# OSU-Bee-Lab/buzzdetect

Hardware: AMD Instinct MI355X
Metric: yamnet_windows_per_s (higher is better)
Workload: dtype f32 (split-f16x3 MFMA products, f32 accumulate)

## Files before the change

### buzzdetect_amd/csrc/bd_device.h

```cpp
#pragma once

#include "bd_internal.h"

#include <mutex>
#include <type_traits>
#ifdef BD_KERNEL_TRACE
#include <cstdio>
#include <cstdlib>
#endif

namespace bd {

namespace {

typedef float f32x16 __attribute__((ext_vector_type(16)));
typedef float v2f __attribute__((ext_vector_type(2)));
typedef float v4f __attribute__((ext_vector_type(4)));
typedef unsigned v4u __attribute__((ext_vector_type(4)));
typedef unsigned u32x2 __attribute__((ext_vector_type(2)));
typedef _Float16 f16x2 __attribute__((ext_vector_type(2)));
typedef _Float16 f16x4 __attribute__((ext_vector_type(4)));
typedef _Float16 f16x8 __attribute__((ext_vector_type(8)));

constexpr float kF16Max = 65504.0f;
__device__ __forceinline__ float range_of(float m, float4 v) {
    return fmaxf(fmaxf(m, fabsf(v.x)), fmaxf(fmaxf(fabsf(v.y), fabsf(v.z)), fabsf(v.w)));
}
__device__ __forceinline__ float range_of(float m, v4f v) {
    return fmaxf(fmaxf(m, fabsf(v.x)), fmaxf(fmaxf(fabsf(v.y), fabsf(v.z)), fabsf(v.w)));
}
__device__ __forceinline__ void range_report(float m, unsigned* __restrict__ flag) {
    if (flag && !(m <= kF16Max)) *flag = 1u;
}

__device__ __forceinline__ int swz64(int row, int slot) { return row * 64 + ((slot ^ ((row >> 2) & 3)) << 4); }

__device__ __forceinline__ void split_f16(float x, float y, float z, float w, f16x4& hi, f16x4& lo) {
    const f16x2 h0 = {(_Float16)x, (_Float16)y}, h1 = {(_Float16)z, (_Float16)w};
    f16x2 l0, l1;
    asm("v_fma_mixlo_f16 %0, %1, -1.0, %2 op_sel:[0,0,0] op_sel_hi:[1,0,0]" : "=v"(l0) : "v"(h0), "v"(x));
    asm("v_fma_mixhi_f16 %0, %1, -1.0, %2 op_sel:[1,0,0] op_sel_hi:[1,0,0]" : "+v"(l0) : "v"(h0), "v"(y));
    asm("v_fma_mixlo_f16 %0, %1, -1.0, %2 op_sel:[0,0,0] op_sel_hi:[1,0,0]" : "=v"(l1) : "v"(h1), "v"(z));
    asm("v_fma_mixhi_f16 %0, %1, -1.0, %2 op_sel:[1,0,0] op_sel_hi:[1,0,0]" : "+v"(l1) : "v"(h1), "v"(w));
    hi[0] = h0[0]; hi[1] = h0[1]; hi[2] = h1[0]; hi[3] = h1[1];
    lo[0] = l0[0]; lo[1] = l0[1]; lo[2] = l1[0]; lo[3] = l1[1];
}
__device__ __forceinline__ void split_f16(v4f a, f16x4& hi, f16x4& lo) { split_f16(a.x, a.y, a.z, a.w, hi, lo); }

constexpr int kTrRowBytes = 192, kTrHalfBytes = 32 * kTrRowBytes, kTrSlotBytes = 2 * kTrHalfBytes;
__host__ __device__ constexpr int tr_image_off(int half, int k, int chunk) {
    return half * kTrHalfBytes + k * kTrRowBytes + ((chunk ^ ((k >> 1) & 7)) << 3);
}
__host__ __device__ constexpr int tr_read_k(int s, int h, int r, int q) { return 16 * s + 8 * h + 4 * r + q; }
__host__ __device__ constexpr int tr_read_chunk(int i, int gp, int p) { return 8 * i + 4 * gp + p; }
constexpr bool tr_image_is_bijection() {
    bool seen[kTrSlotBytes / 8] = {};
    for (int half = 0; half < 2; ++half)
        for (int k = 0; k < 32; ++k)
            for (int t = 0; t < 24; ++t) {
                const int o = tr_image_off(half, k, t);
                if (o < 0 || o >= kTrSlotBytes || o % 8 || seen[o / 8]) return false;
                seen[o / 8] = true;
            }
    return true;
}
constexpr bool tr_image_writes_conflict_free() {
    for (int half = 0; half < 2; ++half)
        for (int a = 0; a < 2; ++a)
            for (int t = 0; t < 24; ++t) {
                unsigned banks = 0;
                for (int l = 0; l < 16; ++l)
                    for (int d = 0; d < 2; ++d) {
                        const unsigned b = 1u << ((tr_image_off(half, 16 * a + l, t) / 4 + d) % 32);
                        if (banks & b) return false;
                        banks |= b;
                    }
            }
    return true;
}
constexpr bool tr_image_reads_conflict_free() {
    for (int half = 0; half < 2; ++half)
        for (int i = 0; i < 3; ++i)
            for (int s = 0; s < 2; ++s)
                for (int h = 0; h < 2; ++h)
                    for (int r = 0; r < 2; ++r) {
                        unsigned long long banks = 0;
                        for (int gp = 0; gp < 2; ++gp)
                            for (int q = 0; q < 4; ++q)
                                for (int p = 0; p < 4; ++p)
                                    for (int d = 0; d < 2; ++d) {
                                        const unsigned long long b =
                                            1ull << ((tr_image_off(half, tr_read_k(s, h, r, q), tr_read_chunk(i, gp, p)) / 4 + d) % 64);
                                        if (banks & b) return false;
                                        banks |= b;
                                    }
                    }
    return true;
}
static_assert(tr_image_is_bijection(), "every (half, k, chunk) has its own 8 bytes of the slot, and they fill it");
static_assert(tr_image_writes_conflict_free(), "a lane group of the publication meets no bank twice");
static_assert(tr_image_reads_conflict_free(), "a lane half of the transposed read meets no bank twice");
__device__ __forceinline__ int tr_read_lane_off(int lane) {
    const int g = lane >> 4, q = (lane >> 2) & 3, p = lane & 3;
    return tr_image_off(0, tr_read_k(0, g >> 1, 0, q), tr_read_chunk(0, g & 1, p));
}
__host__ __device__ constexpr int tr_read_next(int off) { return (off ^ 16) + 4 * kTrRowBytes; }
constexpr bool tr_read_next_holds() {
    for (int lane = 0; lane < 64; ++lane) {
        const int g = lane >> 4, q = (lane >> 2) & 3, p = lane & 3;
        if (tr_read_next(tr_image_off(0, tr_read_k(0, g >> 1, 0, q), tr_read_chunk(0, g & 1, p))) !=
            tr_image_off(0, tr_read_k(0, g >> 1, 1, q), tr_read_chunk(0, g & 1, p)))
            return false;
        for (int s = 0; s < 2; ++s)
            for (int i = 0; i < 3; ++i)
                for (int r = 0; r < 2; ++r)
                    if (tr_image_off(0, tr_read_k(s, g >> 1, r, q), tr_read_chunk(i, g & 1, p)) !=
                        tr_image_off(0, tr_read_k(0, g >> 1, r, q), tr_read_chunk(0, g & 1, p)) + 16 * s * kTrRowBytes + 64 * i)
                        return false;
    }
    return true;
}
static_assert(tr_read_next_holds(), "the reader's immediates");
__device__ __forceinline__ f16x8 tr_read_frag(const char* p0, const char* p1) {
    typedef short s16x4 __attribute__((ext_vector_type(4)));
    typedef __attribute__((address_space(3))) s16x4* lds4;
    const s16x4 a = __builtin_amdgcn_ds_read_tr16_b64_v4i16((lds4)p0), b = __builtin_amdgcn_ds_read_tr16_b64_v4i16((lds4)p1);
    return __builtin_bit_cast(f16x8, __builtin_shufflevector(a, b, 0, 1, 2, 3, 4, 5, 6, 7));
}

__device__ __forceinline__ unsigned pw_lds_addr(const void* p) {
    return (unsigned)(unsigned long long)(__attribute__((address_space(3))) const void*)p;
}
template <int OFFSET>
__device__ __forceinline__ f16x8 pw_lds_frag(unsigned addr) {
    f16x8 v;
    asm volatile("ds_read_b128 %0, %1 offset:%2" : "=v"(v) : "v"(addr), "n"(OFFSET) : "memory");
    return v;
}
__device__ __forceinline__ void pw_lds_store64(unsigned addr, f16x4 v) {
    asm volatile("ds_write_b64 %0, %1" ::"v"(addr), "v"(v) : "memory");
}
__device__ __forceinline__ f16x8 pw_landed(f16x8 v) {
    asm volatile("" : "+v"(v));
    return v;
}
template <int N>
__device__ __forceinline__ void pw_lds_wait() {
    asm volatile("s_waitcnt lgkmcnt(%0)" ::"n"(N) : "memory");
}
template <int I, int E, typename F>
__device__ __forceinline__ void static_for_pw(F&& f) {
    if constexpr (I < E) {
        f(std::integral_constant<int, I>{});
        static_for_pw<I + 1, E>(f);
    }
}
template <int K16, int V, int R>
struct PwResSchedule {
    static constexpr int split_at(int q) {
        for (int j = 0; j < V; ++j)
            if (q == j * K16 / (V > 0 ? V : 1) + 1) return j;
        return -1;
    }
    static constexpr int issued_at_step(int u) { return (u + 2 < K16 ? R : 0) + (split_at(u) >= 0 ? R : 0); }
    static constexpr int pending(int q) {
        int upto_wait = 2 * R;
        for (int u = 0; u <= q; ++u) upto_wait += issued_at_step(u);
        int through_read = q < 2 ? R * (q + 1) : 2 * R;
        if (q >= 2) {
            for (int u = 0; u < q - 2; ++u) through_read += issued_at_step(u);
            through_read += R;
        }
        return upto_wait - through_read;
    }
};

constexpr int kMaxDevices = 64;
template <auto Kernel>
void allow_dynamic_lds(int bytes) {
    static std::once_flag once[kMaxDevices];
    int dev = 0;
    (void)hipGetDevice(&dev);
    std::call_once(once[dev & (kMaxDevices - 1)], [&] {
        (void)hipFuncSetAttribute(reinterpret_cast<const void*>(Kernel), hipFuncAttributeMaxDynamicSharedMemorySize, bytes);
    });
}

#ifdef BD_KERNEL_TRACE
constexpr int kTraceStamps = 128;
template <typename Kernel, typename Launch, typename... Args>
const unsigned long long* traced_launch(char key, Kernel kernel, int lds_bytes, hipStream_t stream, int per_group, int id1,
                                        bool* printed, Launch&& launch, const char* legend, Args... args) {
    const char* tr = getenv("BD_WS_TRACE");
    if (!tr || tr[0] != key) return nullptr;
    static unsigned long long* dbg = nullptr;
    static unsigned long long h[kTraceStamps];
    static int shots = 0;
    if (!dbg) (void)hipMalloc(&dbg, sizeof(h));
    (void)hipFuncSetAttribute(reinterpret_cast<const void*>(kernel), hipFuncAttributeMaxDynamicSharedMemorySize, lds_bytes);
    (void)hipMemsetAsync(dbg, 0, sizeof(h), stream);
    launch(dbg);
    (void)hipStreamSynchronize(stream);
    (void)hipMemcpy(h, dbg, sizeof(h), hipMemcpyDeviceToHost);
    const bool print = ++shots == 8;
    if (printed) *printed = print;
    if (print)
        for (int w = 0; w < 2; ++w) {
            fprintf(stderr, "[trace] ");
            fprintf(stderr, legend, w ? id1 : 0, args...);
            for (int i = 1; i < per_group && h[w * per_group + i]; ++i) fprintf(stderr, " %llu", h[w * per_group + i] - h[w * per_group + i - 1]);
            fprintf(stderr, "\n");
        }
    return h;
}
#endif

}

}
```

### buzzdetect_amd/csrc/l4window.hip

```cpp
#include "bd_device.h"

namespace bd {

namespace {

template <bool PLAIN, bool PLANES>
__global__ __launch_bounds__(768) void l4_window_kernel(
    const float* __restrict__ X, const float* __restrict__ dw_w, const float* __restrict__ dw_b,
    const _Float16* __restrict__ Wfhi, const _Float16* __restrict__ Wflo, const float* __restrict__ pw_u,
    const float* __restrict__ pw_b,
    const float* __restrict__ ndw_w, const float* __restrict__ ndw_b, float* __restrict__ out, int windows,
    unsigned* __restrict__ range_flag, const _Float16* __restrict__ W3fhi, const _Float16* __restrict__ W3flo,
    const float* __restrict__ pw3_u, const float* __restrict__ pw3_b) {
    constexpr int H = 24, W = 16, C = 128, K16 = 8, STEPS = H / 2;
    constexpr int COL_B = C * 4;
    constexpr int ROW_B = (W + 1) * COL_B;
    constexpr int RING0 = COL_B;
    constexpr int A0 = RING0 + 8 * ROW_B;
    constexpr int A_HALF = 32 * 2 * C, A_BUF = 2 * A_HALF;
    constexpr int T5 = A0 + 2 * A_BUF;
    constexpr int O5 = T5 + C * 12 * 4;
    constexpr int O5_ROW = (W / 2) * C * 4, O5_BUF = 2 * O5_ROW;
    constexpr int PL0 = O5 + 2 * O5_BUF;
    constexpr int PL_B = 8192, PL_HALF = 4096;
    constexpr int W3L = PL0 + 2 * PL_B;
    constexpr size_t WIN_IN = (size_t)H * W * C, WIN_OUT = (size_t)STEPS * (W / 2) * C;
    static_assert(A0 % 512 == 0, "fragment addresses are formed by XOR");
    static_assert((2 * STEPS) % 8 == 0 && STEPS % 2 == 0, "ring slots and buffer parities carry over from window to window");
    extern __shared__ __attribute__((aligned(1024))) char smem_raw[];
    char* const smem = smem_raw;
    const int tid = threadIdx.x, lane = tid & 63;
    const int wave = __builtin_amdgcn_readfirstlane(tid >> 6);
    const int b = blockIdx.x, G = gridDim.x;
    if (b >= windows) return;
    const int NT = STEPS * ((windows - b + G - 1) / G);

    for (int i = tid; i < 9 * 32; i += 768) {
        const int z = i >> 5;
        *reinterpret_cast<v4f*>(smem + (z == 0 ? 0 : RING0 + (z - 1) * ROW_B + W * COL_B) + (i & 31) * 16) = v4f{0.f, 0.f, 0.f, 0.f};
    }
    for (int i = tid; i < 10 * C; i += 768) {
        const int t = i / C, c = i - t * C;
        reinterpret_cast<float*>(smem + T5)[c * 12 + t] = t < 9 ? ndw_w[t * C + c] : ndw_b[c];
    }
    float rmax = 0.0f;

    if (wave < 4) {
        const int frow = lane & 31, fh = lane >> 5;
        const int c4 = tid & 31, col_lo = tid >> 5;
        const float* const xt = X + (size_t)b * WIN_IN + (size_t)col_lo * C + c4 * 4;
        char* const ring_t = smem + RING0 + col_lo * COL_B + c4 * 16;
        v4f rs[2][4];
#define BD_L4_LOAD(DST, J)                                                                                \
    {                                                                                                     \
        const int i_ = (J) / STEPS, j_ = (J) - i_ * STEPS;                                                \
        const float* const src_ = xt + (size_t)i_ * G * WIN_IN + (size_t)j_ * (2 * W * C);                \
        _Pragma("unroll") for (int u = 0; u < 4; ++u)                                                     \
            DST[u] = *reinterpret_cast<const v4f*>(src_ + ((u >> 1) * W + 8 * (u & 1)) * C);              \
    }
#define BD_L4_STORE(SRC, J)                                                                               \
    _Pragma("unroll") for (int u = 0; u < 4; ++u)                                                         \
        *reinterpret_cast<v4f*>(ring_t + ((2 * (J) + (u >> 1)) & 7) * ROW_B + 8 * (u & 1) * COL_B) = SRC[u];
        const char* const pt = reinterpret_cast<const char*>(X) + (size_t)b * STEPS * PL_B + tid * 16;
        v4f rp[2], rq[2];
#define BD_L4_PLOAD(DST, J)                                                                               \
    {                                                                                                     \
        const int i_ = (J) / STEPS, j_ = (J) - i_ * STEPS;                                                \
        const char* const src_ = pt + ((size_t)i_ * G * STEPS + j_) * PL_B;                               \
        DST[0] = *reinterpret_cast<const v4f*>(src_);                                                     \
        if constexpr (!PLAIN) DST[1] = *reinterpret_cast<const v4f*>(src_ + PL_HALF);                     \
    }
#define BD_L4_PSTORE(SRC, J)                                                                              \
    {                                                                                                     \
        char* const st_ = smem + PL0 + ((J) & 1) * PL_B + tid * 16;                                       \
        *reinterpret_cast<v4f*>(st_) = SRC[0];                                                            \
        if constexpr (!PLAIN) *reinterpret_cast<v4f*>(st_ + PL_HALF) = SRC[1];                            \
    }
        if constexpr (PLANES) {
            BD_L4_PLOAD(rp, 0)
            BD_L4_PLOAD(rq, 1)
        } else {
            BD_L4_LOAD(rs[0], 0)
            BD_L4_LOAD(rs[1], 1)
        }
        f16x8 bh[K16], bl[K16];
#pragma unroll
        for (int q = 0; q < K16; ++q) {
            const size_t frag = ((size_t)(wave * K16 + q) * 64 + lane) * 8;
            bh[q] = *reinterpret_cast<const f16x8*>(Wfhi + frag);
            if constexpr (!PLAIN) bl[q] = *reinterpret_cast<const f16x8*>(Wflo + frag);
        }
        const int ncol = 32 * wave + frow;
        const float bcol = pw_b[ncol], ucol = pw_u[ncol];
        f16x8 w3h[PLANES ? 4 : 1];
        char* const w3l = smem + W3L + (wave * 4 * 64 + lane) * 16;
        float u3 = 0.0f, b3 = 0.0f;
        if constexpr (PLANES) {
#pragma unroll
            for (int q = 0; q < 4; ++q) {
                const size_t frag = ((size_t)(wave * 4 + q) * 64 + lane) * 8;
                w3h[q] = *reinterpret_cast<const f16x8*>(W3fhi + frag);
                if constexpr (!PLAIN) *reinterpret_cast<f16x8*>(w3l + q * 1024) = *reinterpret_cast<const f16x8*>(W3flo + frag);
            }
            u3 = pw3_u[ncol];
            b3 = pw3_b[ncol];
        }
        typedef const __attribute__((address_space(3))) f16x8* lptrh;
        unsigned pl_a[2];
        pl_a[0] = pw_lds_addr(smem) + (unsigned)(PL0 + frow * 64 + ((fh ^ ((frow >> 2) & 3)) << 4));
        pl_a[1] = pl_a[0] ^ 32u;
        asm("" : "+v"(pl_a[0]), "+v"(pl_a[1]));
        auto pw3 = [&](auto stage_c, int J) {
            constexpr int stage = decltype(stage_c)::value;
            f32x16 acc3;
#pragma unroll
            for (int r = 0; r < 16; ++r) acc3[r] = 0.0f;
#pragma unroll
            for (int q = 0; q < 4; ++q) {
                const unsigned a = pl_a[q & 1] + (unsigned)(stage * PL_B + (q >> 1) * 2048);
                const f16x8 ah = *(lptrh)(size_t)a;
                if constexpr (!PLAIN) {
                    const f16x8 al = *(lptrh)(size_t)(a + PL_HALF);
                    acc3 = __builtin_amdgcn_mfma_f32_32x32x16_f16(al, w3h[q], acc3, 0, 0, 0);
                    acc3 = __builtin_amdgcn_mfma_f32_32x32x16_f16(ah, *reinterpret_cast<const f16x8*>(w3l + q * 1024), acc3, 0, 0, 0);
                }
                acc3 = __builtin_amdgcn_mfma_f32_32x32x16_f16(ah, w3h[q], acc3, 0, 0, 0);
            }
            char* const rw = smem + RING0 + ncol * 4;
#pragma unroll
            for (int r = 0; r < 16; ++r) {
                const int m = 4 * fh + (r & 3) + 8 * (r >> 2);
                *reinterpret_cast<float*>(rw + ((2 * J + (m >> 4)) & 7) * ROW_B + (m & 15) * COL_B) = fmaxf(fmaf(acc3[r], u3, b3), 0.0f);
            }
        };
        const float* const t5 = reinterpret_cast<const float*>(smem + T5) + ncol * 12;
        float acc5[4] = {0.0f, 0.0f, 0.0f, 0.0f};
        float* const o5 = reinterpret_cast<float*>(smem + O5) + (2 * fh) * C + ncol;
        int s5 = 0;
        if constexpr (PLANES) {
            BD_L4_PSTORE(rp, 0)
            BD_L4_PSTORE(rq, 1)
            BD_L4_PLOAD(rp, 2)
            BD_L4_PLOAD(rq, 3)
        } else {
            BD_L4_STORE(rs[0], 0)
            BD_L4_STORE(rs[1], 1)
            BD_L4_LOAD(rs[0], 2)
            BD_L4_LOAD(rs[1], 3)
        }
#pragma unroll
        for (int q = 0; q < K16; ++q) {
            bh[q] = pw_landed(bh[q]);
            if constexpr (!PLAIN) bl[q] = pw_landed(bl[q]);
        }
        if constexpr (PLANES) {
            __syncthreads();
            pw3(std::integral_constant<int, 0>{}, 0);
            __syncthreads();
            BD_L4_PSTORE(rp, 2)
            rp[0] = rq[0];
            rp[1] = rq[1];
            pw3(std::integral_constant<int, 1>{}, 1);
        }
        const unsigned fr0 = pw_lds_addr(smem) + (unsigned)(A0 + frow * 2 * C + ((fh ^ (frow & 15)) << 4));
        __syncthreads();
        auto step = [&](auto pc, int k) {
            constexpr int p = decltype(pc)::value;
            f32x16 acc;
            if (k >= 1 && k <= NT) {
                const unsigned ab = fr0 + (unsigned)((p ^ 1) * A_BUF);
                using S = PwResSchedule<K16, 0, PLAIN ? 1 : 2>;
#pragma unroll
                for (int e = 0; e < 16; ++e) acc[e] = 0.0f;
                f16x8 fa[3][2];
#pragma unroll
                for (int q = 0; q < 2; ++q) {
                    fa[q][0] = pw_lds_frag<0>(ab ^ (q << 5));
                    if constexpr (!PLAIN) fa[q][1] = pw_lds_frag<A_HALF>(ab ^ (q << 5));
                }
                static_for_pw<0, K16>([&](auto qi) {
                    constexpr int q = decltype(qi)::value;
                    if constexpr (q + 2 < K16) {
                        fa[(q + 2) % 3][0] = pw_lds_frag<0>(ab ^ ((q + 2) << 5));
                        if constexpr (!PLAIN) fa[(q + 2) % 3][1] = pw_lds_frag<A_HALF>(ab ^ ((q + 2) << 5));
                    }
                    pw_lds_wait<S::pending(q)>();
                    const f16x8 ah = pw_landed(fa[q % 3][0]);
                    if constexpr (!PLAIN) {
                        const f16x8 al = pw_landed(fa[q % 3][1]);
                        acc = __builtin_amdgcn_mfma_f32_32x32x16_f16(al, bh[q], acc, 0, 0, 0);
                        acc = __builtin_amdgcn_mfma_f32_32x32x16_f16(ah, bl[q], acc, 0, 0, 0);
                    }
                    acc = __builtin_amdgcn_mfma_f32_32x32x16_f16(ah, bh[q], acc, 0, 0, 0);
                });
            }
            if constexpr (PLANES) {
                if (k + 3 < NT) BD_L4_PSTORE(rp, k + 3)
                if (k + 4 < NT) BD_L4_PLOAD(rp, k + 4)
            } else {
                if (k + 2 < NT) { BD_L4_STORE(rs[p], k + 2) }
                if (k + 4 < NT) BD_L4_LOAD(rs[p], k + 4)
            }
            if (k >= 1 && k <= NT) {
                float y[2][8], nb[2][2];
                const v4f t5a = *reinterpret_cast<const v4f*>(t5), t5b = *reinterpret_cast<const v4f*>(t5 + 4), t5c = *reinterpret_cast<const v4f*>(t5 + 8);
                const float w5[9] = {t5a.x, t5a.y, t5a.z, t5a.w, t5b.x, t5b.y, t5b.z, t5b.w, t5c.x};
                const float b5 = t5c.y;
#pragma unroll
                for (int e = 0; e < 16; ++e) y[e >> 3][e & 7] = fmaxf(fmaf(acc[e], ucol, bcol), 0.0f);
#pragma unroll
                for (int r = 0; r < 2; ++r) {
                    float va = y[r][0], wa = y[r][4], vb = y[r][4], wb = 0.0f;
                    asm("" : "+v"(va), "+v"(wa), "+v"(vb), "+v"(wb));
                    const auto s1 = __builtin_amdgcn_permlane32_swap(__builtin_bit_cast(unsigned, va), __builtin_bit_cast(unsigned, wa), false, false);
                    const auto s2 = __builtin_amdgcn_permlane32_swap(__builtin_bit_cast(unsigned, vb), __builtin_bit_cast(unsigned, wb), false, false);
                    nb[r][0] = __builtin_bit_cast(float, fh ? (unsigned)s1[0] : (unsigned)s1[1]);
                    nb[r][1] = fh ? 0.0f : __builtin_bit_cast(float, (unsigned)s2[1]);
                }
#define BD_L4_IN(R, T, KW) ((T) == 0 ? y[R][KW] : (T) == 1 ? ((KW) < 2 ? y[R][2 + (KW)] : nb[R][0]) : (T) == 2 ? y[R][4 + (KW)] : ((KW) < 2 ? y[R][6 + (KW)] : nb[R][1]))
                float* const orow = o5 + (p ^ 1) * (O5_BUF / 4);
                if (s5 > 0) {
#pragma unroll
                    for (int t = 0; t < 4; ++t) {
#pragma unroll
                        for (int kw = 0; kw < 3; ++kw) acc5[t] = fmaf(BD_L4_IN(0, t, kw), w5[6 + kw], acc5[t]);
                        orow[((t >> 1) * 4 + (t & 1)) * C] = fmaxf(acc5[t], 0.0f);
                    }
                }
#pragma unroll
                for (int t = 0; t < 4; ++t) {
                    acc5[t] = b5;
#pragma unroll
                    for (int kh = 0; kh < 2; ++kh)
#pragma unroll
                        for (int kw = 0; kw < 3; ++kw) acc5[t] = fmaf(BD_L4_IN(kh, t, kw), w5[3 * kh + kw], acc5[t]);
                }
                if (s5 == STEPS - 1) {
#pragma unroll
                    for (int t = 0; t < 4; ++t) {
#pragma unroll
                        for (int kw = 0; kw < 3; ++kw) acc5[t] = fmaf(0.0f, w5[6 + kw], acc5[t]);
                        orow[((W / 2) + (t >> 1) * 4 + (t & 1)) * C] = fmaxf(acc5[t], 0.0f);
                    }
                    s5 = 0;
                } else {
                    ++s5;
                }
#undef BD_L4_IN
            }
            if constexpr (PLANES) {
                if (k + 2 < NT) pw3(pc, k + 2);
            }
            __syncthreads();
        };
        for (int k = 0; k < NT + 2; k += 2) {
            step(std::integral_constant<int, 0>{}, k);
            step(std::integral_constant<int, 1>{}, k + 1);
        }
#undef BD_L4_LOAD
#undef BD_L4_STORE
#undef BD_L4_PLOAD
#undef BD_L4_PSTORE
    } else {
        const int v = wave - 4, c4 = lane & 31;
        const int col = v < 4 ? 2 * (2 * v + (lane >> 5)) : 2 * (2 * (v - 4) + (lane >> 5)) + 1;
        v4f w4[9];
#pragma unroll
        for (int t = 0; t < 9; ++t) w4[t] = *reinterpret_cast<const v4f*>(dw_w + t * C + c4 * 4);
        const v4f b4 = *reinterpret_cast<const v4f*>(dw_b + c4 * 4);
        const char* const xin = smem + RING0 + (col - 1) * COL_B + c4 * 16;
        int a_st[2];
#pragma unroll
        for (int rr = 0; rr < 2; ++rr) {
            const int m = 16 * rr + col;
            a_st[rr] = A0 + m * 2 * C + (((c4 >> 1) ^ (m & 15)) << 4) + (c4 & 1) * 8;
        }
        v4f xr[4][3];
        int s4 = 0;
        const int o_lane = (v & 3) * 64 + lane;
        float* const ot = out + (size_t)b * WIN_OUT + (size_t)o_lane * 4;
        int s5 = 0, i5 = 0;
        if constexpr (PLANES) {
            __syncthreads();
            __syncthreads();
        }
        __syncthreads();
        auto step = [&](auto pc, int k) {
            constexpr int p = decltype(pc)::value;
            if (v < 4 && k >= 2) {
                const char* const ob = smem + O5 + p * O5_BUF + o_lane * 16;
                float* const orow = ot + (size_t)i5 * G * WIN_OUT;
                if (s5 > 0) *reinterpret_cast<v4f*>(orow + (size_t)(s5 - 1) * (W / 2) * C) = *reinterpret_cast<const v4f*>(ob);
                if (s5 == STEPS - 1) {
                    *reinterpret_cast<v4f*>(orow + (size_t)s5 * (W / 2) * C) = *reinterpret_cast<const v4f*>(ob + O5_ROW);
                    s5 = 0;
                    ++i5;
                } else {
                    ++s5;
                }
            }
            if (k < NT) {
                if (s4 == 0) {
#pragma unroll
                    for (int c = 0; c < 3; ++c) {
                        xr[0][c] = v4f{0.f, 0.f, 0.f, 0.f};
                        xr[1][c] = *reinterpret_cast<const v4f*>(xin + c * COL_B);
                    }
                }
                {
                    const char* const r2 = xin + ((2 * k + 1) & 7) * ROW_B;
#pragma unroll
                    for (int c = 0; c < 3; ++c) xr[(2 * p + 2) & 3][c] = *reinterpret_cast<const v4f*>(r2 + c * COL_B);
                }
                if (s4 + 1 < STEPS) {
                    const char* const r3 = xin + ((2 * k + 2) & 7) * ROW_B;
#pragma unroll
                    for (int c = 0; c < 3; ++c) xr[(2 * p + 3) & 3][c] = *reinterpret_cast<const v4f*>(r3 + c * COL_B);
                } else {
#pragma unroll
                    for (int c = 0; c < 3; ++c) xr[(2 * p + 3) & 3][c] = v4f{0.f, 0.f, 0.f, 0.f};
                }
#pragma unroll
                for (int rr = 0; rr < 2; ++rr) {
                    v4f a4 = b4;
#pragma unroll
                    for (int kh = 0; kh < 3; ++kh)
#pragma unroll
                        for (int kw = 0; kw < 3; ++kw)
                            a4 = __builtin_elementwise_fma(xr[(2 * p + rr + kh) & 3][kw], w4[kh * 3 + kw], a4);
                    a4.x = fmaxf(a4.x, 0.0f); a4.y = fmaxf(a4.y, 0.0f); a4.z = fmaxf(a4.z, 0.0f); a4.w = fmaxf(a4.w, 0.0f);
                    rmax = range_of(rmax, a4);
                    f16x4 hi, lo;
                    split_f16(a4.x, a4.y, a4.z, a4.w, hi, lo);
                    *reinterpret_cast<f16x4*>(smem + a_st[rr] + p * A_BUF) = hi;
                    if constexpr (!PLAIN) *reinterpret_cast<f16x4*>(smem + a_st[rr] + p * A_BUF + A_HALF) = lo;
                }
                s4 = s4 + 1 == STEPS ? 0 : s4 + 1;
            }
            __syncthreads();
        };
        for (int k = 0; k < NT + 2; k += 2) {
            step(std::integral_constant<int, 0>{}, k);
            step(std::integral_constant<int, 1>{}, k + 1);
        }
    }
    range_report(rmax, range_flag);
}

template <bool PLAIN, bool PLANES>
void launch_l4_window_form(const float* X, const SepLayer* L3, const SepLayer& L, const SepLayer& next, float* out, int windows,
                           hipStream_t stream) {
    constexpr int lds = 512 + 8 * 17 * 512 + 2 * 2 * 32 * 256 + 128 * 12 * 4 + 2 * 2 * 8 * 128 * 4 + (PLANES ? (PLAIN ? 2 : 4) * 8192 : 0);
    allow_dynamic_lds<&l4_window_kernel<PLAIN, PLANES>>(lds);
    const int grid = windows < 256 ? windows : 256;
    hipLaunchKernelGGL((l4_window_kernel<PLAIN, PLANES>), dim3((unsigned)grid), dim3(768), lds, stream, X, dw_w_of(L), dw_b_of(L),
                       static_cast<const _Float16*>(L.pw_fhi), static_cast<const _Float16*>(L.pw_flo), L.pw_u, L.pw_b, dw_w_of(next),
                       dw_b_of(next), out, windows, L.range_flag,
                       PLANES ? static_cast<const _Float16*>(L3->pw_fhi) : nullptr,
                       PLANES ? static_cast<const _Float16*>(L3->pw_flo) : nullptr, PLANES ? L3->pw_u : nullptr,
                       PLANES ? L3->pw_b : nullptr);
}

void launch_l4_window(const float* X, const SepLayer& L, const SepLayer& next, float* out, int windows, hipStream_t stream) {
    if (L.pw_mode == 2) launch_l4_window_form<true, false>(X, nullptr, L, next, out, windows, stream);
    else launch_l4_window_form<false, false>(X, nullptr, L, next, out, windows, stream);
}

}

bool l4_window_planes_supported(const SepLayer& L3, const SepLayer& L4, const SepLayer& L5) {
    return (L3.pw_mode == 1 || L3.pw_mode == 2) && L4.pw_mode == L3.pw_mode && L3.stride == 2 && L3.cin == 64 &&
           L3.cout == 128 && L3.h_out == 24 && L3.w_out == 16 && L3.pw_fhi && L3.pw_flo && L4.stride == 1 && L4.h_out == 24 &&
           L4.w_out == 16 && L4.cin == 128 && L4.cout == 128 && L5.stride == 2 && L5.cin == 128;
}

bool launch_l4_window_planes(const void* planes, const SepLayer& L3, const SepLayer& L4, const SepLayer& L5, float* out,
                             int windows, hipStream_t stream) {
    if (windows <= 0 || !l4_window_planes_supported(L3, L4, L5)) return false;
    const float* const X = static_cast<const float*>(planes);
    if (L4.pw_mode == 2) launch_l4_window_form<true, true>(X, &L3, L4, L5, out, windows, stream);
    else launch_l4_window_form<false, true>(X, &L3, L4, L5, out, windows, stream);
    return true;
}

bool launch_l4_window_next_dw(const float* in, float* out, int windows, const SepLayer& L, const SepLayer& next, hipStream_t stream) {
    if (L.stride != 1 || next.stride != 2 || windows <= 0 || L.h_out * L.w_out != 384 || L.w_out != 16 || L.cin != 128 ||
        L.cout != 128 || next.cin != 128)
        return false;
    launch_l4_window(in, L, next, out, windows, stream);
    return true;
}

}
```

### buzzdetect_amd/csrc/stemreg.hip

```cpp
#include "bd_device.h"

#include <type_traits>

namespace bd {

namespace {

constexpr int OFF_C1 = 0;
constexpr int OFF_AH = 6 * 34 * 32 * 4;
constexpr int OFF_AL = OFF_AH + 128 * 64;
constexpr int OFF_A3H = OFF_AL + 128 * 64;
constexpr int OFF_A3L = OFF_A3H + 2 * 32 * 64;
constexpr int OFF_HALO = OFF_C1 + (2 * 34 + 1) * 32 * 4;
constexpr int OFF_D2W = OFF_A3L + 2 * 32 * 64;
constexpr int OFF_C1W = OFF_D2W + 10 * 32 * 4;
constexpr int kRegLds = OFF_C1W + 10 * 32 * 4;

template <bool PLAIN, bool END_DW3>
__global__ __launch_bounds__(256, 3) void stem_reg_kernel(const float* __restrict__ logmel, int patch_step, const WindowMap map, int w0,
                                                          const float* __restrict__ c1_w, const float* __restrict__ c1_b,
                                                          const float* __restrict__ dw2_w, const float* __restrict__ dw2_b,
                                                          const _Float16* __restrict__ Whi, const _Float16* __restrict__ Wlo,
                                                          const float* __restrict__ pw_u, const float* __restrict__ pw_b,
                                                          const float* __restrict__ dw3_w, const float* __restrict__ dw3_b,
                                                          void* __restrict__ out, const _Float16* __restrict__ W3fhi,
                                                          const _Float16* __restrict__ W3flo, const float* __restrict__ pw3_u,
                                                          const float* __restrict__ pw3_b, unsigned* __restrict__ range_flag, int windows) {
    __shared__ __attribute__((aligned(16))) char smem[kRegLds];
    float (*s_lm)[68] = reinterpret_cast<float (*)[68]>(smem + OFF_AH);
    float (*s_c1)[34][32] = reinterpret_cast<float (*)[34][32]>(smem + OFF_C1);
    char* const s_ah = smem + OFF_AH;
    char* const s_al = smem + OFF_AL;
    float* const s_halo = reinterpret_cast<float*>(smem + OFF_HALO);
    const float* const s_d2 = reinterpret_cast<const float*>(smem + OFF_D2W);
    const float* const s_c1w = reinterpret_cast<const float*>(smem + OFF_C1W);

    const int tid = threadIdx.x, lane = tid & 63, wave = tid >> 6;
    const int c4 = tid & 7, col = tid >> 3;
    const int g = wave >> 1, wc = wave & 1;
    const int frow = lane & 31, fh = lane >> 5;
    float rmax = 0.0f;

    typedef const __attribute__((address_space(1))) float* gptr;
    typedef const __attribute__((address_space(1))) v4f* gptr4;
    typedef const __attribute__((address_space(1))) f16x8* gptrh;
    gptr pc1w = (gptr)c1_w, pc1b = (gptr)c1_b, pd2w = (gptr)dw2_w, pd2b = (gptr)dw2_b, pu2 = (gptr)pw_u, pb2 = (gptr)pw_b,
         pd3w = (gptr)dw3_w, pd3b = (gptr)dw3_b, pu3 = (gptr)pw3_u, pb3 = (gptr)pw3_b;
    const __attribute__((address_space(1))) _Float16 *pwh = (const __attribute__((address_space(1))) _Float16*)Whi,
                                                    *pwl = (const __attribute__((address_space(1))) _Float16*)Wlo,
                                                    *pw3h = (const __attribute__((address_space(1))) _Float16*)W3fhi,
                                                    *pw3l = (const __attribute__((address_space(1))) _Float16*)W3flo;

    const long long total = 12ll * windows;
    const int t_begin = (int)(blockIdx.x * total / gridDim.x), t_end = (int)((blockIdx.x + 1) * total / gridDim.x);

    float4 lmv;
    bool lm_ok = false;
    auto prefetch = [&](int win, int r_first) {
        const float* patch = logmel + window_frame(map, w0 + win, patch_step) * BD_MEL_BANDS;
        const int j = tid >> 4, q = tid & 15;
        const int ih = 2 * r_first - 2 + j;
        lm_ok = j < 13 && ih >= 0 && ih < BD_PATCH_FRAMES;
        const int ihc = ih < 0 ? 0 : ih >= BD_PATCH_FRAMES ? BD_PATCH_FRAMES - 1 : ih;
        lmv = reinterpret_cast<const float4*>(patch + ihc * BD_MEL_BANDS)[q];
    };

    auto band_to_lds = [&](int lmr) {
        if (tid < lmr * 16) {
            float4 v = lmv;
            if (!lm_ok) v = make_float4(0.f, 0.f, 0.f, 0.f);
            *reinterpret_cast<float4*>(&s_lm[tid >> 4][(tid & 15) * 4]) = v;
        } else if (tid >= 256 - lmr) {
            float z;
            asm volatile("v_mov_b32 %0, 0" : "=v"(z));
            *reinterpret_cast<float4*>(&s_lm[255 - tid][64]) = make_float4(z, z, z, z);
        }
    };

    v2f ev[2][8];
    auto front = [&](auto rows_c, int r_first, int c1_new) {
        constexpr int ROWS = decltype(rows_c)::value;
        constexpr int C1R = ROWS + 2;
        v4f c1wt[9];
#pragma unroll
        for (int t = 0; t < 9; ++t) c1wt[t] = *reinterpret_cast<const v4f*>(s_c1w + t * 32 + c4 * 4);
        const v4f c1bias = *reinterpret_cast<const v4f*>(s_c1w + 9 * 32 + c4 * 4);
        {
            float lm[3][3];
            const v4f zero4 = {0.f, 0.f, 0.f, 0.f};
#pragma unroll
            for (int kw = 0; kw < 3; ++kw) lm[0][kw] = s_lm[0][2 * col + kw];
#pragma unroll
            for (int i = 0; i < C1R; ++i) {
                if (i >= c1_new) break;
                const int c1r = r_first - 1 + i;
                float (*const c1row)[32] = s_c1[i];
#pragma unroll
                for (int kh = 1; kh < 3; ++kh)
#pragma unroll
                    for (int kw = 0; kw < 3; ++kw) lm[kh][kw] = s_lm[2 * i + kh][2 * col + kw];
                if (c1r >= 0 && c1r < 48) {
                    v4f acc = c1bias;
#pragma unroll
                    for (int kh = 0; kh < 3; ++kh) {
                        if (2 * c1r + kh >= BD_PATCH_FRAMES) continue;
#pragma unroll
                        for (int kw = 0; kw < 3; ++kw) {
                            const float v = lm[kh][kw];
                            acc = __builtin_elementwise_fma(v4f{v, v, v, v}, c1wt[kh * 3 + kw], acc);
                        }
                    }
                    v4f r4;
                    r4.x = fmaxf(acc.x, 0.0f);
                    r4.y = fmaxf(acc.y, 0.0f);
                    r4.z = fmaxf(acc.z, 0.0f);
                    r4.w = fmaxf(acc.w, 0.0f);
                    *reinterpret_cast<v4f*>(&c1row[col + 1][c4 * 4]) = r4;
                } else {
                    *reinterpret_cast<v4f*>(&c1row[col + 1][c4 * 4]) = zero4;
                }
#pragma unroll
                for (int kw = 0; kw < 3; ++kw) lm[0][kw] = lm[2][kw];
            }
        }
        __syncthreads();
        f16x8 wbh[2], wbl[2];
#pragma unroll
        for (int s2 = 0; s2 < 2; ++s2) {
            const int koff = (wc * 32 + frow) * 32 + (2 * s2 + fh) * 8;
            wbh[s2] = *(gptrh)(pwh + koff);
            wbl[s2] = *(gptrh)(pwl + koff);
        }
        {
            v4f d2wt[9];
#pragma unroll
            for (int t = 0; t < 9; ++t) d2wt[t] = *reinterpret_cast<const v4f*>(s_d2 + t * 32 + c4 * 4);
            const v4f d2bias = *reinterpret_cast<const v4f*>(s_d2 + 9 * 32 + c4 * 4);
            v4f cv[3][3];
#pragma unroll
            for (int kh = 0; kh < 2; ++kh)
#pragma unroll
                for (int kw = 0; kw < 3; ++kw) cv[kh][kw] = *reinterpret_cast<const v4f*>(&s_c1[kh][col + kw][c4 * 4]);
            const int racc = ((col & 1) << 3) + ((col & 15) >> 1);
            const int rbase = 64 * (col >> 4) + 8 * (racc >> 2) + (racc & 3);
#pragma unroll
            for (int r = 0; r < ROWS; ++r) {
#pragma unroll
                for (int kw = 0; kw < 3; ++kw) cv[2][kw] = *reinterpret_cast<const v4f*>(&s_c1[r + 2][col + kw][c4 * 4]);
                v4f acc = d2bias;
#pragma unroll
                for (int kh = 0; kh < 3; ++kh)
#pragma unroll
                    for (int kw = 0; kw < 3; ++kw) acc = __builtin_elementwise_fma(cv[kh][kw], d2wt[kh * 3 + kw], acc);
                acc.x = fmaxf(acc.x, 0.0f);
                acc.y = fmaxf(acc.y, 0.0f);
                acc.z = fmaxf(acc.z, 0.0f);
                acc.w = fmaxf(acc.w, 0.0f);
                rmax = range_of(rmax, acc);
                f16x4 hi, lo;
                split_f16(acc, hi, lo);
                const int row = rbase + 32 * (r & 1) + 4 * (r >> 1);
                const int off = swz64(row, c4 >> 1) + (c4 & 1) * 8;
                *reinterpret_cast<f16x4*>(s_ah + off) = hi;
                *reinterpret_cast<f16x4*>(s_al + off) = lo;
#pragma unroll
                for (int kw = 0; kw < 3; ++kw) {
                    cv[0][kw] = cv[1][kw];
                    cv[1][kw] = cv[2][kw];
                }
            }
        }
        __syncthreads();
        if constexpr (ROWS == 4) {
            const v4f k0 = *reinterpret_cast<const v4f*>(&s_c1[0][col + 1][c4 * 4]);
            const v4f k1 = *reinterpret_cast<const v4f*>(&s_c1[1][col + 1][c4 * 4]);
            *reinterpret_cast<v4f*>(&s_c1[4][col + 1][c4 * 4]) = k0;
            *reinterpret_cast<v4f*>(&s_c1[5][col + 1][c4 * 4]) = k1;
        }
        const float u2 = pu2[wc * 32 + frow], b2 = pb2[wc * 32 + frow];
        f32x16 acc2[2];
#pragma unroll
        for (int t = 0; t < (ROWS == 1 ? 1 : 2); ++t) {
#pragma unroll
            for (int r = 0; r < 16; ++r) acc2[t][r] = 0.0f;
#pragma unroll
            for (int s2 = 0; s2 < 2; ++s2) {
                const int off = swz64((2 * g + t) * 32 + frow, 2 * s2 + fh);
                const f16x8 ah = *reinterpret_cast<const f16x8*>(s_ah + off);
                const f16x8 al = *reinterpret_cast<const f16x8*>(s_al + off);
                if constexpr (!PLAIN) {
                    acc2[t] = __builtin_amdgcn_mfma_f32_32x32x16_f16(al, wbh[s2], acc2[t], 0, 0, 0);
                    acc2[t] = __builtin_amdgcn_mfma_f32_32x32x16_f16(ah, wbl[s2], acc2[t], 0, 0, 0);
                }
                acc2[t] = __builtin_amdgcn_mfma_f32_32x32x16_f16(ah, wbh[s2], acc2[t], 0, 0, 0);
            }
        }
#pragma unroll
        for (int t = 0; t < (ROWS == 1 ? 1 : 2); ++t)
#pragma unroll
            for (int k = 0; k < 8; ++k) {
                const v2f v = __builtin_elementwise_fma(v2f{acc2[t][2 * k], acc2[t][2 * k + 1]}, v2f{u2, u2}, v2f{b2, b2});
                ev[t][k] = v2f{fmaxf(v.x, 0.0f), fmaxf(v.y, 0.0f)};
            }
    };

    v2f carry[8];
    if (t_begin < t_end) {
        if (tid >= 96 && tid < 96 + 160) {
            const int which = (tid - 96) / 80, row = ((tid - 96) % 80) >> 3, cc = tid & 7;
            gptr w = which ? pd2w : pc1w, bs = which ? pd2b : pc1b;
            *reinterpret_cast<v4f*>(smem + (which ? OFF_D2W : OFF_C1W) + (row * 32 + cc * 4) * 4) = row < 9 ? *(gptr4)(w + row * 32 + cc * 4) : *(gptr4)(bs + cc * 4);
        }
        if (tid < 6 * 2 * 8) {
            const int r = tid / 16, side = (tid >> 3) & 1, cc = tid & 7;
            *reinterpret_cast<float4*>(&s_c1[r][side ? 33 : 0][cc * 4]) = make_float4(0.f, 0.f, 0.f, 0.f);
        }
        {
            const int win0 = t_begin / 12, ob0 = 11 - t_begin % 12;
            if (ob0 != 11) {
                prefetch(win0, 4 * ob0 + 4);
                band_to_lds(7);
                __syncthreads();
                front(std::integral_constant<int, 1>{}, 4 * ob0 + 4, 3);
#pragma unroll
                for (int k = 0; k < 8; ++k) carry[k] = ev[0][k];
                __syncthreads();
            } else {
#pragma unroll
                for (int k = 0; k < 8; ++k) carry[k] = v2f{0.0f, 0.0f};
            }
            prefetch(win0, 4 * ob0);
            band_to_lds(13);
            __syncthreads();
        }
#pragma unroll 1
        for (int t = t_begin; t < t_end; ++t) {
            asm volatile("" : "+s"(pc1w), "+s"(pc1b), "+s"(pd2w), "+s"(pd2b), "+s"(pu2), "+s"(pb2), "+s"(pwh), "+s"(pwl));
            asm volatile("" : "+s"(pd3w), "+s"(pd3b), "+s"(pu3), "+s"(pb3), "+s"(pw3h), "+s"(pw3l));
            const int win = t / 12, ob = 11 - t % 12;
            {
                const int tn = t + 1 < t_end ? t + 1 : t;
                prefetch(tn / 12, 4 * (11 - tn % 12));
            }
            if (ob == 11 && t != t_begin) {
#pragma unroll
                for (int k = 0; k < 8; ++k) carry[k] = v2f{0.0f, 0.0f};
            }
            front(std::integral_constant<int, 4>{}, 4 * ob, (t == t_begin || ob == 11) ? 6 : 4);

            v2f x2[8];
#pragma unroll
            for (int k = 0; k < 8; ++k) {
                float e0 = ev[0][k].x, e1 = ev[0][k].y, c0 = carry[k].x, c1 = carry[k].y;
                asm("" : "+v"(e0), "+v"(e1), "+v"(c0), "+v"(c1));
                const auto s0 = __builtin_amdgcn_permlane32_swap(__builtin_bit_cast(unsigned, e0), __builtin_bit_cast(unsigned, c0), false, false);
                const auto s1 = __builtin_amdgcn_permlane32_swap(__builtin_bit_cast(unsigned, e1), __builtin_bit_cast(unsigned, c1), false, false);
                x2[k] = v2f{__builtin_bit_cast(float, fh ? (unsigned)s0[0] : (unsigned)s0[1]),
                            __builtin_bit_cast(float, fh ? (unsigned)s1[0] : (unsigned)s1[1])};
            }
            if (g == 1) {
                float* const hw = s_halo + ((wc * 2 + fh) * 3) * 32 + frow;
                hw[0] = ev[0][0].x;
                hw[32] = ev[1][0].x;
                hw[64] = x2[0].x;
            }
            float d3w[9];
#pragma unroll
            for (int k = 0; k < 9; ++k) d3w[k] = pd3w[k * 64 + wc * 32 + frow];
            const float d3b = pd3b[wc * 32 + frow];
            f16x8 w3h[4], w3l[4];
            if constexpr (!END_DW3) {
#pragma unroll
                for (int q = 0; q < 4; ++q) w3h[q] = *(gptrh)(pw3h + ((size_t)(wave * 4 + q) * 64 + lane) * 8);
            }
            __syncthreads();
            band_to_lds(13);
            float hal[3] = {0.0f, 0.0f, 0.0f};
            if (g == 0) {
                const float* const hr = s_halo + ((wc * 2 + fh) * 3) * 32 + frow;
                hal[0] = hr[0];
                hal[1] = hr[32];
                hal[2] = hr[64];
            }
#pragma unroll
            for (int k = 0; k < 4; ++k) {
                v2f a = v2f{d3b, d3b};
#pragma unroll
                for (int kh = 0; kh < 3; ++kh) {
                    const v2f* const row = kh == 0 ? ev[0] : kh == 1 ? ev[1] : x2;
                    v2f shifted;
                    if (k < 3) asm("v_pk_mov_b32 %0, %1, %2 op_sel:[1,0]" : "=v"(shifted) : "v"(row[k]), "v"(row[k < 3 ? k + 1 : 0]));
                    else shifted = v2f{row[k].y, hal[kh]};
                    a = __builtin_elementwise_fma(row[k], v2f{d3w[kh * 3], d3w[kh * 3]}, a);
                    a = __builtin_elementwise_fma(row[4 + k], v2f{d3w[kh * 3 + 1], d3w[kh * 3 + 1]}, a);
                    a = __builtin_elementwise_fma(shifted, v2f{d3w[kh * 3 + 2], d3w[kh * 3 + 2]}, a);
                }
                {
                    const float v0 = fmaxf(a.x, 0.0f), v1 = fmaxf(a.y, 0.0f);
                    unsigned pkh, pkl;
                    asm volatile("v_cvt_pk_f16_f32 %0, %3, %4\n\t"
                                 "v_fma_mixlo_f16 %1, %0, -1.0, %3 op_sel:[0,0,0] op_sel_hi:[1,0,0]\n\t"
                                 "v_fma_mixhi_f16 %1, %0, -1.0, %4 op_sel:[1,0,0] op_sel_hi:[1,0,0]\n\t"
                                 "v_max3_f32 %2, %2, %3, %4"
                                 : "=&v"(pkh), "=&v"(pkl), "+v"(rmax) : "v"(v0), "v"(v1));
                    const int off0 = wc * (32 * 64) + swz64(fh * 16 + 8 * g + 2 * k, frow >> 3) + (frow & 7) * 2;
                    const int off1 = wc * (32 * 64) + swz64(fh * 16 + 8 * g + 2 * k + 1, frow >> 3) + (frow & 7) * 2;
                    *reinterpret_cast<unsigned short*>(smem + OFF_A3H + off0) = (unsigned short)pkh;
                    *reinterpret_cast<unsigned short*>(smem + OFF_A3H + off1) = (unsigned short)(pkh >> 16);
                    *reinterpret_cast<unsigned short*>(smem + OFF_A3L + off0) = (unsigned short)pkl;
                    *reinterpret_cast<unsigned short*>(smem + OFF_A3L + off1) = (unsigned short)(pkl >> 16);
                }
            }
#pragma unroll
            for (int k = 0; k < 8; ++k) carry[k] = ev[0][k];
            if constexpr (END_DW3) {
                __syncthreads();
                typedef __attribute__((address_space(1))) char* gchar;
                const gchar dst = (gchar)out + ((size_t)win * 12 + ob) * 8192 + tid * 16;
                const v4f ph = *reinterpret_cast<const v4f*>(smem + OFF_A3H + tid * 16);
                asm volatile("global_store_dwordx4 %0, %1, off\n\ts_nop 2" : : "v"(dst), "v"(ph) : "memory");
                if constexpr (!PLAIN) {
                    const v4f pl = *reinterpret_cast<const v4f*>(smem + OFF_A3L + tid * 16);
                    asm volatile("global_store_dwordx4 %0, %1, off\n\ts_nop 2" : : "v"(dst + 4096), "v"(pl) : "memory");
                }
            } else {
                if constexpr (!PLAIN) {
#pragma unroll
                    for (int q = 0; q < 4; ++q) w3l[q] = *(gptrh)(pw3l + ((size_t)(wave * 4 + q) * 64 + lane) * 8);
                }
                const int n3 = 32 * wave + frow;
                const float b3 = pb3[n3], u3 = pu3[n3];
                __syncthreads();
                f32x16 acc3;
#pragma unroll
                for (int r = 0; r < 16; ++r) acc3[r] = 0.0f;
#pragma unroll
                for (int q = 0; q < 4; ++q) {
                    const int off = (q >> 1) * 32 * 64 + swz64(frow, 2 * (q & 1) + fh);
                    const f16x8 ah = *reinterpret_cast<const f16x8*>(smem + OFF_A3H + off);
                    const f16x8 al = *reinterpret_cast<const f16x8*>(smem + OFF_A3L + off);
                    if constexpr (!PLAIN) {
                        acc3 = __builtin_amdgcn_mfma_f32_32x32x16_f16(al, w3h[q], acc3, 0, 0, 0);
                        acc3 = __builtin_amdgcn_mfma_f32_32x32x16_f16(ah, w3l[q], acc3, 0, 0, 0);
                    }
                    acc3 = __builtin_amdgcn_mfma_f32_32x32x16_f16(ah, w3h[q], acc3, 0, 0, 0);
                }
                float* dst3 = static_cast<float*>(out) + (((size_t)win * 24 + 2 * ob) * 16) * 128;
#pragma unroll
                for (int r = 0; r < 16; ++r) {
                    const int m = 4 * fh + (r & 3) + 8 * (r >> 2);
                    const v2f t2v = __builtin_elementwise_fma(v2f{acc3[r & ~1], acc3[r | 1]}, v2f{u3, u3}, v2f{b3, b3});
                    dst3[(size_t)m * 128 + n3] = fmaxf((r & 1) ? t2v.y : t2v.x, 0.0f);
                }
            }
        }
    }
    range_report(rmax, range_flag);
}

}

static void launch_stem_reg_form(const float* logmel, int patch_step, const WindowMap& map, int w0, int windows, const float* c1_w,
                                 const float* c1_b, const SepLayer& L2, const SepLayer& L3, void* out, hipStream_t stream,
                                 bool planes) {
    if (windows <= 0) return;
    long long grid = 3ll * cu_count();
    if (grid > 12ll * windows) grid = 12ll * windows;
#define BD_STEM_REG(PLAIN, END_DW3)                                                                                  \
    hipLaunchKernelGGL((stem_reg_kernel<PLAIN, END_DW3>), dim3((unsigned)grid), dim3(256), 0, stream, logmel, patch_step, map, w0,   \
                       c1_w, c1_b, dw_w_of(L2), dw_b_of(L2), static_cast<const _Float16*>(L2.pw_whi),                     \
                       static_cast<const _Float16*>(L2.pw_wlo), L2.pw_u, L2.pw_b, dw_w_of(L3), dw_b_of(L3), out,            \
                       static_cast<const _Float16*>(L3.pw_fhi), static_cast<const _Float16*>(L3.pw_flo), L3.pw_u, L3.pw_b,  \
                       L2.range_flag, windows)
    if (planes) {
        if (L2.pw_mode == 2) BD_STEM_REG(true, true);
        else BD_STEM_REG(false, true);
    } else {
        if (L2.pw_mode == 2) BD_STEM_REG(true, false);
        else BD_STEM_REG(false, false);
    }
#undef BD_STEM_REG
}

void launch_stem_reg(const float* logmel, int patch_step, const WindowMap& map, int w0, int windows, const float* c1_w,
                     const float* c1_b, const SepLayer& L2, const SepLayer& L3, float* out, hipStream_t stream) {
    launch_stem_reg_form(logmel, patch_step, map, w0, windows, c1_w, c1_b, L2, L3, out, stream, false);
}

void launch_stem_reg_planes(const float* logmel, int patch_step, const WindowMap& map, int w0, int windows, const float* c1_w,
                            const float* c1_b, const SepLayer& L2, const SepLayer& L3, float* out, hipStream_t stream) {
    launch_stem_reg_form(logmel, patch_step, map, w0, windows, c1_w, c1_b, L2, L3, out, stream, true);
}

}
```

Measured before the change: 2.104 million.

## Store dw3 planes directly from registers in a k-major layout read via transposed LDS loads

The stem kernel's END_DW3 path used to scatter per-element f16 results into an LDS tile, sync, then copy 16-byte chunks to global memory. It now packs each lane's four results into registers and writes them straight to global memory in a new k-major plane layout, removing the scattered LDS stores and a block barrier. The l4 window kernel stages these planes into LDS with an XOR swizzle and reads them with ds_read_tr16_b64 transposed loads, and static_asserts check the swizzle is bijective and free of bank conflicts. The logmel band load is moved earlier and relocated into the freed tile, which may change the overlap between stages.

New measurement: 2.060 million. 0.979x the previous value.

```diff
diff --git a/buzzdetect_amd/csrc/bd_device.h b/buzzdetect_amd/csrc/bd_device.h
--- a/buzzdetect_amd/csrc/bd_device.h
+++ b/buzzdetect_amd/csrc/bd_device.h
@@ -127,6 +127,77 @@
     const s16x4 a = __builtin_amdgcn_ds_read_tr16_b64_v4i16((lds4)p0), b = __builtin_amdgcn_ds_read_tr16_b64_v4i16((lds4)p1);
     return __builtin_bit_cast(f16x8, __builtin_shufflevector(a, b, 0, 1, 2, 3, 4, 5, 6, 7));
 }
+__device__ __forceinline__ f16x8 tr_read_frag(unsigned a0, unsigned a1) {
+    typedef short s16x4 __attribute__((ext_vector_type(4)));
+    typedef __attribute__((address_space(3))) s16x4* lds4;
+    const s16x4 a = __builtin_amdgcn_ds_read_tr16_b64_v4i16((lds4)(size_t)a0), b = __builtin_amdgcn_ds_read_tr16_b64_v4i16((lds4)(size_t)a1);
+    return __builtin_bit_cast(f16x8, __builtin_shufflevector(a, b, 0, 1, 2, 3, 4, 5, 6, 7));
+}
+
+constexpr int kDw3PlaneBytes = 4096, kDw3PairBytes = 2 * kDw3PlaneBytes;
+__host__ __device__ constexpr int dw3_plane_off(int k, int y, int x) {
+    return ((k >> 5) * 2 + (x >> 3)) * 1024 + (k & 31) * 32 + y * 16 + (x & 7) * 2;
+}
+__host__ __device__ constexpr int dw3_stage_off(int plane_off) { return plane_off ^ ((plane_off >> 3) & 128); }
+__host__ __device__ constexpr int dw3_read_k(int s, int h, int r, int q) { return 16 * s + 8 * h + 4 * r + q; }
+__host__ __device__ constexpr int dw3_read_lane_off(int lane) {
+    return dw3_stage_off(dw3_plane_off(dw3_read_k(0, lane >> 5, 0, (lane >> 2) & 3), (lane >> 4) & 1, 4 * (lane & 3)));
+}
+constexpr bool dw3_stage_is_bijection() {
+    bool seen[kDw3PlaneBytes / 8] = {};
+    for (int k = 0; k < 64; ++k)
+        for (int y = 0; y < 2; ++y)
+            for (int x = 0; x < 16; x += 4) {
+                const int o = dw3_stage_off(dw3_plane_off(k, y, x));
+                if (o < 0 || o >= kDw3PlaneBytes || o % 8 || seen[o / 8]) return false;
+                if (dw3_stage_off(dw3_plane_off(k, y, x + 3)) != o + 6) return false;
+                seen[o / 8] = true;
+            }
+    for (int piece = 0; piece < kDw3PlaneBytes; piece += 16)
+        if (dw3_stage_off(piece) % 16 || dw3_stage_off(piece + 15) != dw3_stage_off(piece) + 15) return false;
+    return true;
+}
+constexpr bool dw3_stage_copy_conflict_free() {
+    for (int t0 = 0; t0 < kDw3PlaneBytes / 16; t0 += 8) {
+        unsigned banks = 0;
+        for (int l = 0; l < 8; ++l)
+            for (int d = 0; d < 4; ++d) {
+                const unsigned b = 1u << ((dw3_stage_off((t0 + l) * 16) / 4 + d) % 32);
+                if (banks & b) return false;
+                banks |= b;
+            }
+    }
+    return true;
+}
+constexpr bool dw3_stage_reads_conflict_free() {
+    for (int s = 0; s < 4; ++s)
+        for (int h = 0; h < 2; ++h)
+            for (int r = 0; r < 2; ++r) {
+                unsigned long long banks = 0;
+                for (int y = 0; y < 2; ++y)
+                    for (int q = 0; q < 4; ++q)
+                        for (int p = 0; p < 4; ++p)
+                            for (int d = 0; d < 2; ++d) {
+                                const unsigned long long b = 1ull << ((dw3_stage_off(dw3_plane_off(dw3_read_k(s, h, r, q), y, 4 * p)) / 4 + d) % 64);
+                                if (banks & b) return false;
+                                banks |= b;
+                            }
+            }
+    return true;
+}
+constexpr bool dw3_read_immediates_hold() {
+    for (int lane = 0; lane < 64; ++lane)
+        for (int s = 0; s < 4; ++s)
+            for (int r = 0; r < 2; ++r)
+                if (dw3_stage_off(dw3_plane_off(dw3_read_k(s, lane >> 5, r, (lane >> 2) & 3), (lane >> 4) & 1, 4 * (lane & 3))) !=
+                    (dw3_read_lane_off(lane) ^ (128 * r)) + 512 * (s & 1) + 2048 * (s >> 1))
+                    return false;
+    return true;
+}
+static_assert(dw3_stage_is_bijection(), "every (k, row, four columns) has its own 8 bytes of the stage's plane, and they fill it");
+static_assert(dw3_stage_copy_conflict_free(), "a lane group of the stage copy meets no bank twice");
+static_assert(dw3_stage_reads_conflict_free(), "a lane half of the transposed read meets no bank twice");
+static_assert(dw3_read_immediates_hold(), "the reader's immediates");
 
 __device__ __forceinline__ unsigned pw_lds_addr(const void* p) {
     return (unsigned)(unsigned long long)(__attribute__((address_space(3))) const void*)p;
diff --git a/buzzdetect_amd/csrc/l4window.hip b/buzzdetect_amd/csrc/l4window.hip
--- a/buzzdetect_amd/csrc/l4window.hip
+++ b/buzzdetect_amd/csrc/l4window.hip
@@ -62,6 +62,7 @@
     _Pragma("unroll") for (int u = 0; u < 4; ++u)                                                         \
         *reinterpret_cast<v4f*>(ring_t + ((2 * (J) + (u >> 1)) & 7) * ROW_B + 8 * (u & 1) * COL_B) = SRC[u];
         const char* const pt = reinterpret_cast<const char*>(X) + (size_t)b * STEPS * PL_B + tid * 16;
+        char* const pst = smem + PL0 + dw3_stage_off(tid * 16);
         v4f rp[2], rq[2];
 #define BD_L4_PLOAD(DST, J)                                                                               \
     {                                                                                                     \
@@ -72,7 +73,7 @@
     }
 #define BD_L4_PSTORE(SRC, J)                                                                              \
     {                                                                                                     \
-        char* const st_ = smem + PL0 + ((J) & 1) * PL_B + tid * 16;                                       \
+        char* const st_ = pst + ((J) & 1) * PL_B;                                                         \
         *reinterpret_cast<v4f*>(st_) = SRC[0];                                                            \
         if constexpr (!PLAIN) *reinterpret_cast<v4f*>(st_ + PL_HALF) = SRC[1];                            \
     }
@@ -105,10 +106,10 @@
             u3 = pw3_u[ncol];
             b3 = pw3_b[ncol];
         }
-        typedef const __attribute__((address_space(3))) f16x8* lptrh;
+        static_assert(PL_B == kDw3PairBytes && PL_HALF == kDw3PlaneBytes, "the stage holds the stem's planes of a row pair");
         unsigned pl_a[2];
-        pl_a[0] = pw_lds_addr(smem) + (unsigned)(PL0 + frow * 64 + ((fh ^ ((frow >> 2) & 3)) << 4));
-        pl_a[1] = pl_a[0] ^ 32u;
+        pl_a[0] = pw_lds_addr(smem) + (unsigned)(PL0 + dw3_read_lane_off(lane));
+        pl_a[1] = pw_lds_addr(smem) + (unsigned)(PL0 + (dw3_read_lane_off(lane) ^ 128));
         asm("" : "+v"(pl_a[0]), "+v"(pl_a[1]));
         auto pw3 = [&](auto stage_c, int J) {
             constexpr int stage = decltype(stage_c)::value;
@@ -117,10 +118,10 @@
             for (int r = 0; r < 16; ++r) acc3[r] = 0.0f;
 #pragma unroll
             for (int q = 0; q < 4; ++q) {
-                const unsigned a = pl_a[q & 1] + (unsigned)(stage * PL_B + (q >> 1) * 2048);
-                const f16x8 ah = *(lptrh)(size_t)a;
+                const unsigned o =stage * PL_B + (q >> 1) * 2048 + (q & 1) * 512;
+                const f16x8 ah = tr_read_frag(pl_a[0] + o, pl_a[1] + o);
                 if constexpr (!PLAIN) {
-                    const f16x8 al = *(lptrh)(size_t)(a + PL_HALF);
+                    const f16x8 al = tr_read_frag(pl_a[0] + o + PL_HALF, pl_a[1] + o + PL_HALF);
                     acc3 = __builtin_amdgcn_mfma_f32_32x32x16_f16(al, w3h[q], acc3, 0, 0, 0);
                     acc3 = __builtin_amdgcn_mfma_f32_32x32x16_f16(ah, *reinterpret_cast<const f16x8*>(w3l + q * 1024), acc3, 0, 0, 0);
                 }
diff --git a/buzzdetect_amd/csrc/stemreg.hip b/buzzdetect_amd/csrc/stemreg.hip
--- a/buzzdetect_amd/csrc/stemreg.hip
+++ b/buzzdetect_amd/csrc/stemreg.hip
@@ -15,6 +15,9 @@
 constexpr int OFF_D2W = OFF_A3L + 2 * 32 * 64;
 constexpr int OFF_C1W = OFF_D2W + 10 * 32 * 4;
 constexpr int kRegLds = OFF_C1W + 10 * 32 * 4;
+constexpr int OFF_LM_DW3 = OFF_A3H;
+constexpr int OFF_HALO_DW3 = OFF_A3H + 3584;
+static_assert(OFF_LM_DW3 + 13 * 68 * 4 <= OFF_HALO_DW3 && OFF_HALO_DW3 + 2 * 2 * 3 * 32 * 4 <= OFF_D2W, "the band and the halo fit the freed tile");
 
 template <bool PLAIN, bool END_DW3>
 __global__ __launch_bounds__(256, 3) void stem_reg_kernel(const float* __restrict__ logmel, int patch_step, const WindowMap map, int w0,
@@ -27,11 +30,11 @@
                                                           const _Float16* __restrict__ W3flo, const float* __restrict__ pw3_u,
                                                           const float* __restrict__ pw3_b, unsigned* __restrict__ range_flag, int windows) {
     __shared__ __attribute__((aligned(16))) char smem[kRegLds];
-    float (*s_lm)[68] = reinterpret_cast<float (*)[68]>(smem + OFF_AH);
+    float (*s_lm)[68] = reinterpret_cast<float (*)[68]>(smem + (END_DW3 ? OFF_LM_DW3 : OFF_AH));
     float (*s_c1)[34][32] = reinterpret_cast<float (*)[34][32]>(smem + OFF_C1);
     char* const s_ah = smem + OFF_AH;
     char* const s_al = smem + OFF_AL;
-    float* const s_halo = reinterpret_cast<float*>(smem + OFF_HALO);
+    float* const s_halo = reinterpret_cast<float*>(smem + (END_DW3 ? OFF_HALO_DW3 : OFF_HALO));
     const float* const s_d2 = reinterpret_cast<const float*>(smem + OFF_D2W);
     const float* const s_c1w = reinterpret_cast<const float*>(smem + OFF_C1W);
 
@@ -171,6 +174,7 @@
             }
         }
         __syncthreads();
+        if constexpr (END_DW3 && ROWS == 4) band_to_lds(13);
         if constexpr (ROWS == 4) {
             const v4f k0 = *reinterpret_cast<const v4f*>(&s_c1[0][col + 1][c4 * 4]);
             const v4f k1 = *reinterpret_cast<const v4f*>(&s_c1[1][col + 1][c4 * 4]);
@@ -274,7 +278,7 @@
                 for (int q = 0; q < 4; ++q) w3h[q] = *(gptrh)(pw3h + ((size_t)(wave * 4 + q) * 64 + lane) * 8);
             }
             __syncthreads();
-            band_to_lds(13);
+            if constexpr (!END_DW3) band_to_lds(13);
             float hal[3] = {0.0f, 0.0f, 0.0f};
             if (g == 0) {
                 const float* const hr = s_halo + ((wc * 2 + fh) * 3) * 32 + frow;
@@ -282,6 +286,8 @@
                 hal[1] = hr[32];
                 hal[2] = hr[64];
             }
+            typedef unsigned u32x4 __attribute__((ext_vector_type(4)));
+            u32x4 ph, pl;
 #pragma unroll
             for (int k = 0; k < 4; ++k) {
                 v2f a = v2f{d3b, d3b};
@@ -303,26 +309,26 @@
                                  "v_fma_mixhi_f16 %1, %0, -1.0, %4 op_sel:[1,0,0] op_sel_hi:[1,0,0]\n\t"
                                  "v_max3_f32 %2, %2, %3, %4"
                                  : "=&v"(pkh), "=&v"(pkl), "+v"(rmax) : "v"(v0), "v"(v1));
-                    const int off0 = wc * (32 * 64) + swz64(fh * 16 + 8 * g + 2 * k, frow >> 3) + (frow & 7) * 2;
-                    const int off1 = wc * (32 * 64) + swz64(fh * 16 + 8 * g + 2 * k + 1, frow >> 3) + (frow & 7) * 2;
-                    *reinterpret_cast<unsigned short*>(smem + OFF_A3H + off0) = (unsigned short)pkh;
-                    *reinterpret_cast<unsigned short*>(smem + OFF_A3H + off1) = (unsigned short)(pkh >> 16);
-                    *reinterpret_cast<unsigned short*>(smem + OFF_A3L + off0) = (unsigned short)pkl;
-                    *reinterpret_cast<unsigned short*>(smem + OFF_A3L + off1) = (unsigned short)(pkl >> 16);
+                    if constexpr (END_DW3) {
+                        ph[k] = pkh;
+                        pl[k] = pkl;
+                    } else {
+                        const int off0 = wc * (32 * 64) + swz64(fh * 16 + 8 * g + 2 * k, frow >> 3) + (frow & 7) * 2;
+                        const int off1 = wc * (32 * 64) + swz64(fh * 16 + 8 * g + 2 * k + 1, frow >> 3) + (frow & 7) * 2;
+                        *reinterpret_cast<unsigned short*>(smem + OFF_A3H + off0) = (unsigned short)pkh;
+                        *reinterpret_cast<unsigned short*>(smem + OFF_A3H + off1) = (unsigned short)(pkh >> 16);
+                        *reinterpret_cast<unsigned short*>(smem + OFF_A3L + off0) = (unsigned short)pkl;
+                        *reinterpret_cast<unsigned short*>(smem + OFF_A3L + off1) = (unsigned short)(pkl >> 16);
+                    }
                 }
             }
 #pragma unroll
             for (int k = 0; k < 8; ++k) carry[k] = ev[0][k];
             if constexpr (END_DW3) {
-                __syncthreads();
                 typedef __attribute__((address_space(1))) char* gchar;
-                const gchar dst = (gchar)out + ((size_t)win * 12 + ob) * 8192 + tid * 16;
-                const v4f ph = *reinterpret_cast<const v4f*>(smem + OFF_A3H + tid * 16);
+                const gchar dst = (gchar)out + ((size_t)win * 12 + ob) * kDw3PairBytes + dw3_plane_off(32 * wc + frow, fh, 8 * g);
                 asm volatile("global_store_dwordx4 %0, %1, off\n\ts_nop 2" : : "v"(dst), "v"(ph) : "memory");
-                if constexpr (!PLAIN) {
-                    const v4f pl = *reinterpret_cast<const v4f*>(smem + OFF_A3L + tid * 16);
-                    asm volatile("global_store_dwordx4 %0, %1, off\n\ts_nop 2" : : "v"(dst + 4096), "v"(pl) : "memory");
-                }
+                if constexpr (!PLAIN) asm volatile("global_store_dwordx4 %0, %1, off\n\ts_nop 2" : : "v"(dst + kDw3PlaneBytes), "v"(pl) : "memory");
             } else {
                 if constexpr (!PLAIN) {
 #pragma unroll
```
